# NHLBI/long_context_biomedical_imaging

Hardware: AMD Instinct MI355X
Metric: image-tokens/sec fwd+bwd, ViT patch=2 512^2 (L=65536), 1/2/4/8 MI355X (higher is better)
Workload: dtype bf16; 1 GPU; ViT-small p2 512x512 2-D seg (ViTUNETR head), full attention; global_batch=2, seq_len=65536, parallelism=ddp1, per_gpu_batch=2, optimizer=adam, loss=CrossEntropy, activation_checkpointing=none, hip_graph=False, tuned_gemms=True

## Files before the change

include/lci.h:

```cpp
#ifndef LCI_H_
#define LCI_H_

#ifdef __cplusplus
extern "C" {
#endif

#define LCI_ABI_VERSION 37
const char* lci_last_error(void);
int lci_abi_version(void);
const char* lci_build_hash(void);

int lci_attn_fwd(const void* qkv, void* out, float* lse2, float* knorm_ws, int B, int L, int H, int head_dim,
                 float scale, void* stream);
long long lci_attn_fwd_ws_bytes(int B, int L, int H);
int lci_attn_fwd_variant(int variant, const void* qkv, void* out, float* lse2, float* knorm_ws, int B, int L, int H,
                         int head_dim, float scale, void* stream);
int lci_attn_fwd_pick(int B, int L, int H, int n_cu);
int lci_attn_bwd(const void* qkv, const void* out, const void* dout, const float* lse2, void* dqkv,
                 float* delta_ws, int B, int L, int H, int head_dim, float scale, void* stream);
long long lci_attn_bwd_ws_bytes(int B, int H, int L);
int lci_attn_bwd_stage(int stage, const void* qkv, const void* out, const void* dout, const float* lse2,
                       void* dqkv, float* delta_ws, int B, int L, int H, int head_dim, float scale, void* stream);
int lci_attn_bwd_variant(int dq_variant, int stage, const void* qkv, const void* out, const void* dout,
                         const float* lse2, void* dqkv, float* delta_ws, int B, int L, int H, int head_dim,
                         float scale, void* stream);
int lci_attn_bwd_dq_pick(int B, int L, int H, int n_cu);

int lci_attn_gen_fwd(int dtype, const void* qkv, void* out, float* lse, int B, int L, int H, int head_dim,
                     float scale, void* stream);
int lci_attn_gen_bwd(int dtype, const void* qkv, const void* out, const void* dout, const float* lse, void* dqkv,
                     float* delta_ws, int B, int L, int H, int head_dim, float scale, void* stream);

long long lci_window_bias_elems(const int* geo, int has_mask);
int lci_window_bias(const float* rpb, const float* mask, void* bias, void* biasT, const int* geo, void* stream);
int lci_window_attn_fwd(const void* qkv, const float* qkv_bias, const void* biasT, int has_mask, void* out,
                        float* lse2, const int* geo, float scale, void* stream);
int lci_window_attn_bwd(const void* qkv, const float* qkv_bias, const void* bias, const void* biasT, int has_mask,
                        const void* out, const void* dout, const float* lse2, void* dqkv, float* dbias_pad,
                        float* pad_ws, void* dS, float* drpb, const int* geo, float scale, void* stream);
long long lci_window_dS_elems(const int* geo);
long long lci_window_pad_ws_elems(const int* geo);
int lci_window_bwd_needs_plain(const int* geo);
int lci_window_index_map(const int* geo, int* src_row, int* region, int* rid, int* wtype, void* stream);

int lci_window_gather(const void* src, void* dst, int elem_bytes, const int* geo, int scatter, void* stream);

int lci_conv3_fwd(const void* x, const void* w, void* y, int B, int D, int H, int W, int Cin, int Cout, int KD,
                  void* stream);
int lci_conv3_fwd_splits(long long V, int Cin, int Cout, int KD);
// ... 158 lines not shown
```

long_context_biomedical_imaging_amd/_lib.py:

```python
from __future__ import annotations

import ctypes
import os

import torch

HERE = os.path.dirname(os.path.abspath(__file__))
DEFAULT_LIB = os.path.join(HERE, "liblci.so")
LIB_PATH = os.environ.get("LCI_LIB_PATH", DEFAULT_LIB)
ABI_VERSION = 37

_P = ctypes.c_void_p
_I = ctypes.c_int
_F = ctypes.c_float
_L = ctypes.c_longlong
_D = ctypes.c_double

SIGNATURES = {
    "lci_attn_fwd": [_P, _P, _P, _P, _I, _I, _I, _I, _F, _P],
    "lci_attn_fwd_variant": [_I, _P, _P, _P, _P, _I, _I, _I, _I, _F, _P],
    "lci_attn_bwd": [_P, _P, _P, _P, _P, _P, _I, _I, _I, _I, _F, _P],
    "lci_attn_bwd_stage": [_I, _P, _P, _P, _P, _P, _P, _I, _I, _I, _I, _F, _P],
    "lci_attn_bwd_variant": [_I, _I, _P, _P, _P, _P, _P, _P, _I, _I, _I, _I, _F, _P],
    "lci_attn_gen_fwd": [_I, _P, _P, _P, _I, _I, _I, _I, _F, _P],
    "lci_attn_gen_bwd": [_I, _P, _P, _P, _P, _P, _P, _I, _I, _I, _I, _F, _P],
    "lci_patch_embed_fwd": [_P, _I, _P, _P, _P, _P, _I, _I, _I, _I, _I, _P, _P, _I, _P],
    "lci_patch_embed_bwd": [_P, _I, _P, _I, _P, _P, _P, _I, _I, _I, _I, _P, _P, _I, _P],
    "lci_selective_scan_fwd": [_I, _P, _P, _P, _P, _P, _P, _P, _P, _P, _I, _I, _I, _I, _I, _I, _P, _P, _P, _P, _P],
    "lci_selective_scan_bwd": [_I, _P, _P, _P, _P, _P, _P, _P, _P, _P, _P, _P, _P, _P, _P, _P, _I, _I, _I, _I, _I,
                               _I, _P, _P, _P, _P, _P],
    "lci_window_bias": [_P, _P, _P, _P, _P, _P],
    "lci_window_attn_fwd": [_P, _P, _P, _I, _P, _P, _P, _F, _P],
    "lci_window_attn_bwd": [_P, _P, _P, _P, _I, _P, _P, _P, _P, _P, _P, _P, _P, _P, _F, _P],
    "lci_window_index_map": [_P, _P, _P, _P, _P, _P],
    "lci_fft_twiddles": [_P, _I, _P],
    "lci_fftconv_spectrum": [_P, _P, _P, _P, _P, _I, _I, _P],
    "lci_fftconv_fwd": [_P, _P, _P, _P, _P, _P, _P, _I, _I, _I, _P],
    "lci_fftconv_bwd": [_P, _P, _P, _P, _P, _P, _P, _P, _P, _P, _P, _P, _I, _I, _I, _P],
    "lci_hyena_pre_fwd": [_I, _P, _P, _P, _P, _P, _I, _I, _I, _I, _I, _P],
    "lci_hyena_post_fwd": [_I, _P, _P, _P, _I, _I, _I, _P],
    "lci_hyena_post_bwd": [_I, _P, _P, _P, _P, _P, _I, _I, _I, _P],
    "lci_hyena_pre_bwd": [_I, _P, _P, _P, _P, _P, _P, _P, _P, _I, _I, _I, _I, _I, _P],
    "lci_dwconv_silu_fwd": [_I, _P, _P, _P, _P, _P, _P, _P, _I, _I, _I, _I, _I, _I, _I, _I, _P],
    "lci_conv3_fwd": [_P, _P, _P, _I, _I, _I, _I, _I, _I, _I, _P],
    "lci_conv3_fwd_split": [_P, _P, _P, _P, _I, _I, _I, _I, _I, _I, _I, _I, _P],
    "lci_conv3_pack_weight": [_P, _P, _I, _I, _I, _I, _I, _P],
# ... 61 lines not shown
    lib.lci_abi_version.restype = ctypes.c_int
    lib.lci_build_hash.restype = ctypes.c_char_p
    if lib.lci_abi_version() != ABI_VERSION:
        raise LciError(f"{path}: ABI version {lib.lci_abi_version()} != {ABI_VERSION} expected by this binding; "
                       "rebuild with `python -m long_context_biomedical_imaging_amd.build_lib`")
    if path == DEFAULT_LIB and os.path.isdir(os.path.join(HERE, "csrc")):
        from . import build_lib
        want, got = build_lib.source_hash(), lib.lci_build_hash().decode()
        if want != got:
            raise LciError(f"{path} is stale: built from sources {got}, the sources beside it hash to {want}; "
                           "rebuild with `python -m long_context_biomedical_imaging_amd.build_lib`")
    lib.lci_window_dS_elems.restype = ctypes.c_longlong
    lib.lci_window_dS_elems.argtypes = [_P]
    lib.lci_window_pad_ws_elems.restype = ctypes.c_longlong
    lib.lci_window_pad_ws_elems.argtypes = [_P]
    lib.lci_window_bwd_needs_plain.restype = ctypes.c_int
    lib.lci_window_bwd_needs_plain.argtypes = [_P]
    lib.lci_selective_scan_bwd_plain_dbc.restype = ctypes.c_int
    lib.lci_selective_scan_bwd_plain_dbc.argtypes = [_I, _I, _I]
    lib.lci_window_bias_elems.restype = ctypes.c_longlong
    lib.lci_window_bias_elems.argtypes = [_P, _I]
    lib.lci_attn_bwd_ws_bytes.restype = ctypes.c_longlong
    lib.lci_attn_bwd_ws_bytes.argtypes = [_I, _I, _I]
    lib.lci_attn_fwd_ws_bytes.restype = ctypes.c_longlong
    lib.lci_attn_fwd_ws_bytes.argtypes = [_I, _I, _I]
    lib.lci_attn_fwd_pick.restype = ctypes.c_int
    lib.lci_attn_fwd_pick.argtypes = [_I, _I, _I, _I]
    lib.lci_attn_bwd_dq_pick.restype = ctypes.c_int
    lib.lci_attn_bwd_dq_pick.argtypes = [_I, _I, _I, _I]
    lib.lci_conv3_fwd_splits.restype = ctypes.c_int
    lib.lci_conv3_fwd_splits.argtypes = [ctypes.c_longlong, _I, _I, _I]
    lib.lci_conv3_wgrad_splits.restype = ctypes.c_longlong
    lib.lci_conv3_wgrad_splits.argtypes = [ctypes.c_longlong, _I, _I, _I]
    lib.lci_linear_wgrad_splits.restype = ctypes.c_longlong
    lib.lci_linear_wgrad_splits.argtypes = [ctypes.c_longlong, _I, _I]
    lib.lci_gemm_bt_supported.restype = ctypes.c_int
    lib.lci_gemm_bt_supported.argtypes = [_I, _I]
    lib.lci_gemm_bt_small_supported.restype = ctypes.c_int
    lib.lci_gemm_bt_small_supported.argtypes = [_I, _I]
    lib.lci_linear_small_threads.restype = ctypes.c_int
    lib.lci_linear_small_threads.argtypes = []
    lib.lci_inorm_chunks.restype = ctypes.c_int
    lib.lci_inorm_chunks.argtypes = [ctypes.c_longlong, _I]
    lib.lci_layernorm_bwd_blocks.restype = ctypes.c_int
    lib.lci_layernorm_bwd_blocks.argtypes = [ctypes.c_longlong]
    lib.lci_hyena_filter_img_elems.restype = ctypes.c_longlong
    lib.lci_hyena_filter_img_elems.argtypes = []
    lib.lci_hyena_filter_partials.restype = ctypes.c_longlong
    lib.lci_hyena_filter_partials.argtypes = [_I, _I]
    lib.lci_fft_size.restype = ctypes.c_longlong
    lib.lci_fft_size.argtypes = [_I]
    lib.lci_dwconv_silu_bwd_part_rows.restype = ctypes.c_longlong
# ... 52 lines not shown
```

long_context_biomedical_imaging_amd/csrc/attention.hip:

```cpp
#include "common.hpp"

#include <type_traits>
#include <utility>

namespace lci {

constexpr int DH = 64;
constexpr int KT = 64;
constexpr float NEG_BIG = -1.0e30f;

struct AttnArgs {
  const bf16* q; const bf16* k; const bf16* v;
  const bf16* o; const bf16* dout;
  bf16* out;
  bf16* dk; bf16* dv;
  float* lse2;
  float* delta;
  long long bs_q, bs_k, bs_v, bs_o, bs_do, bs_out, bs_dk, bs_dv;
  int rs_q, rs_k, rs_v, rs_o, rs_do, rs_out, rs_dk, rs_dv;
  int hs;
  int H, L;
  float c;
  float scale;
};

__global__ __launch_bounds__(256) void attn_key_norm_kernel(AttnArgs a, float* knorm, int nkt) {
  const int lane = threadIdx.x & 63, t = blockIdx.x * 4 + (threadIdx.x >> 6);
  const int hh = blockIdx.y, b = blockIdx.z;
  if (t >= nkt) return;
  const int key = t * KT + lane;
  float ss = 0.f;
  if (key < a.L) {
    const bf16* kp = a.k + b * a.bs_k + (long long)key * a.rs_k + hh * a.hs;
#pragma unroll
    for (int c = 0; c < DH / 8; ++c) {
      const bf16x8 v = *(const bf16x8*)(kp + 8 * c);
#pragma unroll
      for (int j = 0; j < 8; ++j) ss += to_f32(v[j]) * to_f32(v[j]);
    }
  }
#pragma unroll
  for (int off = 32; off >= 1; off >>= 1) ss = fmaxf(ss, __shfl_xor(ss, off));
  if (lane == 0) knorm[((long long)b * a.H + hh) * nkt + t] = sqrtf(ss);
}

constexpr float SAFE_EXP2 = 64.f;
__global__ __launch_bounds__(256) void attn_bwd_delta_kernel(AttnArgs a) {
  const int tid = threadIdx.x;
  const int row = blockIdx.x * 32 + (tid >> 3), ch = tid & 7;
  const int hh = blockIdx.y, b = blockIdx.z;
  float acc = 0.f;
  if (row < a.L) {
    const bf16x8 o = *(const bf16x8*)(a.o + b * a.bs_o + (long long)row * a.rs_o + hh * a.hs + ch * 8);
    const bf16x8 d = *(const bf16x8*)(a.dout + b * a.bs_do + (long long)row * a.rs_do + hh * a.hs + ch * 8);
#pragma unroll
    for (int j = 0; j < 8; ++j) acc += to_f32(o[j]) * to_f32(d[j]);
  }
  acc += __shfl_xor(acc, 1);
  acc += __shfl_xor(acc, 2);
  acc += __shfl_xor(acc, 4);
  if (ch == 0 && row < a.L) {
    float* ws = a.delta + ((long long)b * a.H + hh) * 2 * a.L;
    ws[row] = -a.lse2[((long long)b * a.H + hh) * a.L + row];
    ws[a.L + row] = -acc;
  }
}

constexpr int HS_NW = 4;
__device__ __forceinline__ int sw128(int row, int col) {
  const int g = ((row >> 2) & 3) | (((row >> 1) & 1) << 2);
  return row * DH + ((((col >> 3) ^ g) << 3) | (col & 7));
}
__device__ __forceinline__ void hs_dma16(rsrc_t r, int voff, int soff, unsigned lds) {
  unsigned keep;
  asm volatile("s_mov_b32 %0, m0\n\ts_mov_b32 m0, %3\n\ts_nop 0\n\tbuffer_load_dwordx4 %1, %2, %4 offen lds\n\ts_mov_b32 m0, %0"
               : "=&s"(keep) : "v"(voff), "s"(r), "s"(lds), "s"(soff) : "memory");
}
__device__ __forceinline__ void hs_dma4(rsrc_t r, int voff, int soff, unsigned lds) {
  unsigned keep;
  asm volatile("s_mov_b32 %0, m0\n\ts_mov_b32 m0, %3\n\ts_nop 0\n\tbuffer_load_dword %1, %2, %4 offen lds\n\ts_mov_b32 m0, %0"
               : "=&s"(keep) : "v"(voff), "s"(r), "s"(lds), "s"(soff) : "memory");
}
__device__ __forceinline__ u32x4 hs_ld16(rsrc_t r, int voff, int soff) {
  u32x4 v;
  asm volatile("buffer_load_dwordx4 %0, %1, %2, %3 offen" : "=a"(v) : "v"(voff), "s"(r), "s"(soff) : "memory");
  return v;
}
__device__ __forceinline__ uint32_t hs_ld4(rsrc_t r, int voff, int soff) {
// ... 26 lines not shown
template <int OFF>
__device__ __forceinline__ void hs_st4(unsigned addr, uint32_t v) {
  asm volatile("ds_write_b32 %0, %1 offset:%2" ::"v"(addr), "a"(v), "i"(OFF) : "memory");
}
__device__ __forceinline__ u32x4 hs_ld16v(rsrc_t r, int voff, int soff) {
  u32x4 v;
  asm volatile("buffer_load_dwordx4 %0, %1, %2, %3 offen" : "=v"(v) : "v"(voff), "s"(r), "s"(soff) : "memory");
  return v;
}
template <int OFF>
__device__ __forceinline__ void hs_st16v(unsigned addr, const u32x4& v) {
  asm volatile("ds_write_b128 %0, %1 offset:%2" ::"v"(addr), "v"(v), "i"(OFF) : "memory");
}
template <class F, int... G>
__device__ __forceinline__ void hs_for_gaps(F&& f, std::integer_sequence<int, G...>) {
  (f(std::integral_constant<int, G>{}), ...);
}
#ifndef LCI_DKDV_PROBE
#define LCI_DKDV_PROBE 0
#endif
#ifndef LCI_DKDV_DPPRC
#define LCI_DKDV_DPPRC 0
#endif
template <int I>
__device__ __forceinline__ float hs_bcast(float x) {
  float d;
  asm volatile("v_mov_b32_dpp %0, %1 row_newbcast:%2 row_mask:0xf bank_mask:0xf" : "=v"(d) : "v"(x), "i"(I));
  return d;
}
__device__ __forceinline__ float hs_bcast_i(float x, int i) {
  switch (i & 15) {
    case 0: return hs_bcast<0>(x); case 1: return hs_bcast<1>(x); case 2: return hs_bcast<2>(x);
    case 3: return hs_bcast<3>(x); case 4: return hs_bcast<4>(x); case 5: return hs_bcast<5>(x);
    case 6: return hs_bcast<6>(x); case 7: return hs_bcast<7>(x); case 8: return hs_bcast<8>(x);
    case 9: return hs_bcast<9>(x); case 10: return hs_bcast<10>(x); case 11: return hs_bcast<11>(x);
    case 12: return hs_bcast<12>(x); case 13: return hs_bcast<13>(x); case 14: return hs_bcast<14>(x);
    default: return hs_bcast<15>(x);
  }
}
__global__ __launch_bounds__(HS_NW * 64, 1) void attn_bwd_dkdv_hs_kernel(AttnArgs a) {
  constexpr bool DPPRC = LCI_DKDV_DPPRC != 0;
  constexpr int TILE_B = KT * DH * 2;
  constexpr int SLOT_B = 2 * TILE_B;
  constexpr int RC_B = 2 * KT * 4;
  constexpr int NSLOT = 4;
  constexpr int NOPS = 5;
  static_assert((NSLOT & (NSLOT - 1)) == 0, "ring slot of tile t is t & (NSLOT - 1)");
  static_assert(NSLOT * SLOT_B == 65536, "Q / dO ring reachable by DS immediates");
  __shared__ __attribute__((aligned(16))) char smem[NSLOT * SLOT_B + NSLOT * RC_B];
  char* const rcs = smem + NSLOT * SLOT_B;
  const int tid = threadIdx.x, lane = tid & 63;
  const int wave = __builtin_amdgcn_readfirstlane(tid >> 6);
  const int hh = blockIdx.y, b = blockIdx.z;
  const int L = a.L;
  const int h = lane >> 5, r32 = lane & 31;
  const int kw0 = blockIdx.x * (HS_NW * 64) + wave * 64;
  const int nqt = (L + KT - 1) / KT;

  bf16x8 kf[2][4], vf[2][4];
  {
    const bf16* kp = a.k + b * a.bs_k + hh * a.hs;
    const bf16* vp = a.v + b * a.bs_v + hh * a.hs;
#pragma unroll
    for (int kb = 0; kb < 2; ++kb) {
      const int key = kw0 + 32 * kb + r32;
#pragma unroll
      for (int ks = 0; ks < 4; ++ks) {
        if (key < L) {
          kf[kb][ks] = *(const bf16x8*)(kp + (long long)key * a.rs_k + 16 * ks + 8 * h);
          vf[kb][ks] = *(const bf16x8*)(vp + (long long)key * a.rs_v + 16 * ks + 8 * h);
        } else {
          kf[kb][ks] = bf16x8{};
          vf[kb][ks] = bf16x8{};
        }
#pragma unroll
        for (int j = 0; j < 8; ++j) kf[kb][ks][j] = to_bf16(to_f32(kf[kb][ks][j]) * a.c);
      }
    }
  }
  hs_vmcnt<0>();
#pragma unroll
  for (int i = 0; i < 2; ++i)
#pragma unroll
    for (int j = 0; j < 4; ++j)
      { HS_TO_AGPR(kf[i][j]); HS_TO_AGPR(vf[i][j]); }

  const int rs2q = a.rs_q * 2, rs2d = a.rs_do * 2;
  const rsrc_t rq = make_rsrc(a.q + b * a.bs_q + hh * a.hs, (uint32_t)(L - 1) * (uint32_t)rs2q + DH * 2);
  const rsrc_t rd = make_rsrc(a.dout + b * a.bs_do + hh * a.hs, (uint32_t)(L - 1) * (uint32_t)rs2d + DH * 2);
  const rsrc_t rr = make_rsrc(a.delta + ((long long)b * a.H + hh) * 2 * L + (wave & 1) * L, (uint32_t)L * 4);
  const int prow = lane >> 3;
  const int pch0 = (lane & 7) ^ ((prow >> 2) | ((prow >> 1) & 1) << 2);
  const int pch1 = (lane & 7) ^ ((2 + (prow >> 2)) | ((prow >> 1) & 1) << 2);
  const int dq0 = (16 * wave + prow) * rs2q + 16 * pch0, dq1 = (16 * wave + 8 + prow) * rs2q + 16 * pch1;
  const int dd0 = (16 * wave + prow) * rs2d + 16 * pch0, dd1 = (16 * wave + 8 + prow) * rs2d + 16 * pch1;
  const unsigned lds0 = (unsigned)(uintptr_t)(LCI_LDS char*)smem;
  auto dma_op = [&](int t, int i) __attribute__((always_inline)) {
    const unsigned sb = lds0 + (unsigned)((t & (NSLOT - 1)) * SLOT_B);
    if (i == 0) hs_dma16(rq, dq0, t * KT * rs2q, sb + 2048 * wave);
    if (i == 1) hs_dma16(rq, dq1, t * KT * rs2q, sb + 2048 * wave + 1024);
    if (i == 2) hs_dma16(rd, dd0, t * KT * rs2d, sb + TILE_B + 2048 * wave);
    if (i == 3) hs_dma16(rd, dd1, t * KT * rs2d, sb + TILE_B + 2048 * wave + 1024);
    if (i == 4) hs_dma4(rr, lane * 4, t * KT * 4, lds0 + (unsigned)(NSLOT * SLOT_B + (t & (NSLOT - 1)) * RC_B +
                                                                     (wave & 1) * KT * 4));
  };
  auto dma_tile = [&](int t) __attribute__((always_inline)) {
#pragma unroll
    for (int i = 0; i < NOPS; ++i) dma_op(t, i);
  };
  unsigned q_off[4], t_off[2][2], rc_off;
#pragma unroll
  for (int ks = 0; ks < 4; ++ks) {
    q_off[ks] = 2 * sw128(r32, 16 * ks + 8 * h);
// ... 117 lines not shown
    for (int g = 0; g < 8; ++g) {
      chain_gap(g, 0, ST);
      valu_gap(g, 1, 1, 1, 0);
      if (!(g & 1)) tr_load(g >> 1, C, slot, r0);
      sgap(0, g);
    }
    mid();
#pragma unroll
    for (int g = 0; g < 8; ++g) {
      grad_gap(g, 1, C ^ 1);
      valu_gap(g, 0, 0, 1, 1);
      if (!(g & 1)) tr_load(4 + (g >> 1), C, slot, r0);
      if (DPPRC) {
        if (g == 1) xNL = rcx_load(nrc, 0, nr0);
        if (g == 3) xND = rcx_load(nrc, 1, nr0);
        if (g >= 5) bc_gap(g - 5, NST);
      }
      sgap(1, g);
    }
#pragma unroll
    for (int g = 0; g < 8; ++g) {
      chain_gap(g, 1, ST);
      valu_gap(g, 0, 1, 0, 0);
      if (g == 2) HS_KEEP(NLs[ST]);
      if (g == 6) HS_KEEP(NDs[ST]);
      if (DPPRC) bc_gap(3 + g, NST);
      if (g >= 2 && g < 6) qa[g - 2] = qrow(nslot, nr0, g - 2);
      if (g >= 6) {
        if (!DPPRC) rc_load(NLs[0], nrc, 0, nr0, g - 6);
        da[g - 6] = qrow(nslot + TILE_B, nr0, g - 6);
      }
      sgap(2, g);
    }
#pragma unroll
    for (int g = 0; g < 8; ++g) {
      grad_gap(g, 0, C);
      valu_gap(g, 1, 0, 0, 1);
      if (DPPRC) bc_gap(11 + g, NST);
      if (g < 2) { if (!DPPRC) rc_load(NLs[0], nrc, 0, nr0, g + 2); }
      else if (g < 6) { if (!DPPRC) rc_load(NDs[0], nrc, 1, nr0, g - 2); }
      else da[g - 4] = qrow(nslot + TILE_B, nr0, g - 4);
      sgap(3, g);
    }
  };

  u32x4 rsq[4];
  uint32_t rsr = 0;
  const unsigned wst = lds0 + 2048 * wave + 16 * lane;
  const unsigned wrc = lds0 + NSLOT * SLOT_B + (wave & 1) * KT * 4 + 4 * lane;
  auto ld_piece = [&](int t, int i) __attribute__((always_inline)) {
    if (i == 0) rsq[0] = hs_ld16(rq, dq0, t * KT * rs2q);
    if (i == 1) rsq[1] = hs_ld16(rq, dq1, t * KT * rs2q);
    if (i == 2) rsq[2] = hs_ld16(rd, dd0, t * KT * rs2d);
    if (i == 3) rsq[3] = hs_ld16(rd, dd1, t * KT * rs2d);
    if (i == 4) rsr = hs_ld4(rr, lane * 4, t * KT * 4);
  };
  dma_tile(0);
  ld_piece(1, 0); ld_piece(1, 1); ld_piece(1, 2); ld_piece(1, 3); ld_piece(1, 4);
  hs_vmcnt<0>();
  __syncthreads();
  NLs[0] = rcblk(rcs, 0, 0);
  NDs[0] = rcblk(rcs, 1, 0);
#pragma unroll
  for (int ks = 0; ks < 4; ++ks) {
    qa[ks] = qrow(0, 0, ks);
    da[ks] = qrow(TILE_B, 0, ks);
  }
  __builtin_amdgcn_s_waitcnt(LGKM0_WAIT);
  auto tile = [&](auto SL, int t) __attribute__((always_inline)) {
    constexpr int SLC = decltype(SL)::value;
    const int sl = SLC >= 0 ? SLC : t & (NSLOT - 1), nsl = SLC >= 0 ? (SLC + 1) & (NSLOT - 1) : (t + 1) & (NSLOT - 1);
    const int slot = sl * SLOT_B, nslot = nsl * SLOT_B, rc = sl * RC_B, nrc = nsl * RC_B;
    auto stage = [&]() __attribute__((always_inline)) {
      if (!(LCI_DKDV_PROBE & 1) && t + 1 < nqt) __builtin_amdgcn_s_barrier();
    };
    auto rstg0 = [&](int seg, int g) __attribute__((always_inline)) {
      if (!(g & 1)) return;
      constexpr int SS = 0, LS = 2;
      if (!(LCI_DKDV_PROBE & 2) && seg == SS && g == 1) hs_vmcnt<0>();
      constexpr int S1 = SLC >= 0 ? ((SLC + 1) & (NSLOT - 1)) * SLOT_B : 0;
      constexpr int R1 = SLC >= 0 ? ((SLC + 1) & (NSLOT - 1)) * RC_B : 0;
      const unsigned base = SLC >= 0 ? wst : wst + (unsigned)nslot;
      const unsigned rbase = SLC >= 0 ? wrc : wrc + (unsigned)nrc;
      if (seg == SS) {
// ... 38 lines not shown

  const float sc = a.scale;
#pragma unroll
  for (int kb = 0; kb < 2; ++kb) {
    const int key = kw0 + 32 * kb + r32;
    if (key < L) {
      bf16* dkp = a.dk + b * a.bs_dk + (long long)key * a.rs_dk + hh * a.hs;
      bf16* dvp = a.dv + b * a.bs_dv + (long long)key * a.rs_dv + hh * a.hs;
#pragma unroll
      for (int db = 0; db < 2; ++db)
#pragma unroll
        for (int g = 0; g < 4; ++g) {
          bf16x4 k4, v4;
#pragma unroll
          for (int j = 0; j < 4; ++j) {
            k4[j] = to_bf16(dk[db][kb][4 * g + j] * sc);
            v4[j] = to_bf16(dv[db][kb][4 * g + j]);
          }
          *(bf16x4*)(dkp + 32 * db + 8 * g + 4 * h) = k4;
          *(bf16x4*)(dvp + 32 * db + 8 * g + 4 * h) = v4;
        }
    }
  }
}

constexpr unsigned char DQ_SCHED[24][4] = {
    {0x28, 0x29, 0xff, 0xff},
    {0x68, 0x69, 0x2a, 0xa4},
    {0x6a, 0x2b, 0x2c, 0xff},
    {0x6b, 0x6c, 0xa5, 0x2d},
    {0x2e, 0x6d, 0x2f, 0xa6},
    {0x6e, 0x6f, 0x00, 0xa7},
    {0x01, 0x02, 0xff, 0xff},
    {0x03, 0x04, 0xff, 0xff},
    {0x05, 0x06, 0xff, 0xff},
    {0x40, 0x41, 0x42, 0x43},
    {0x80, 0x81, 0x44, 0x45},
    {0x46, 0x82, 0x07, 0x08},
    {0x47, 0x48, 0x83, 0x09},
    {0x0a, 0x49, 0x0b, 0x84},
    {0x4a, 0x4b, 0x0c, 0x85},
    {0x4c, 0x0d, 0x0e, 0xff},
    {0x4d, 0x4e, 0x86, 0x0f},
    {0x20, 0x4f, 0x21, 0x87},
    {0x22, 0x23, 0xff, 0xff},
    {0x24, 0x25, 0xff, 0xff},
// ... 1590 lines not shown
  hipLaunchKernelGGL(attn_key_norm_kernel, dim3((nkt + 3) / 4, H, B), dim3(256), 0, s, a, knorm_ws, nkt);
  LCI_LAUNCH_CHECK();
  if (variant < 0) variant = lci_attn_fwd_pick(B, L, H, attn_n_cu());
  if (variant == 1)
    hipLaunchKernelGGL(attn_fwd_hs4_kernel, dim3((L + FW4_QWG - 1) / FW4_QWG, H, B), dim3(HS_NW * 64), 0, s, a,
                       (const float*)knorm_ws);
  else
    hipLaunchKernelGGL(attn_fwd_hs_kernel, dim3((L + HS_NW * 64 - 1) / (HS_NW * 64), H, B), dim3(HS_NW * 64), 0, s, a,
                       (const float*)knorm_ws);
  LCI_LAUNCH_CHECK();
  return 0;
}

extern "C" int lci_attn_fwd(const void* qkv, void* out, float* lse2, float* knorm_ws, int B, int L, int H,
                            int head_dim, float scale, void* stream) {
  return lci_attn_fwd_variant(-1, qkv, out, lse2, knorm_ws, B, L, H, head_dim, scale, stream);
}

extern "C" long long lci_attn_bwd_ws_bytes(int B, int H, int L) {
  const long long flags = (long long)B * H * ((L + DQ4_QWG - 1) / DQ4_QWG);
  return ((dq4_flag_offset(B, H, L) + flags) * 4 + 255) / 256 * 256;
}

extern "C" int lci_attn_bwd_variant(int dq_variant, int stage, const void* qkv, const void* out, const void* dout,
                                    const float* lse2, void* dqkv, float* delta_ws, int B, int L, int H, int head_dim,
                                    float scale, void* stream) {
  LCI_CHECK(dq_variant >= -1 && dq_variant <= 1, "lci_attn_bwd_variant: dq_variant %d (want -1, 0 or 1)", dq_variant);
  LCI_CHECK(head_dim == DH, "lci_attn_bwd: head_dim %d unsupported (only 64)", head_dim);
  LCI_CHECK(B > 0 && L > 0 && H > 0, "lci_attn_bwd: bad shape B=%d L=%d H=%d", B, L, H);
  const int rs = 3 * H * DH;
  LCI_CHECK(check_packed(qkv, rs) && check_packed(dqkv, rs) && check_packed(out, H * DH) &&
                check_packed(dout, H * DH), "lci_attn_bwd: misaligned pointers");
  LCI_CHECK((long long)(L + 6 * KT) * rs * 2 < (1ll << 31), "lci_attn_bwd: L=%d too long for 32-bit buffer offsets", L);
  LCI_CHECK(delta_ws != nullptr, "lci_attn_bwd: delta_ws (lci_attn_bwd_ws_bytes) is required");
  AttnArgs a{};
  const bf16* base = (const bf16*)qkv;
  bf16* dbase = (bf16*)dqkv;
  a.q = base; a.k = base + H * DH; a.v = base + 2 * H * DH;
  a.o = (const bf16*)out; a.dout = (const bf16*)dout;
  a.lse2 = (float*)lse2; a.delta = delta_ws;
  a.bs_q = a.bs_k = a.bs_v = (long long)L * rs;
  a.rs_q = a.rs_k = a.rs_v = rs;
  a.bs_o = a.bs_do = (long long)L * H * DH;
  a.rs_o = a.rs_do = H * DH;
  a.out = dbase; a.dk = dbase + H * DH; a.dv = dbase + 2 * H * DH;
  a.bs_out = a.bs_dk = a.bs_dv = (long long)L * rs;
  a.rs_out = a.rs_dk = a.rs_dv = rs;
  a.hs = DH; a.H = H; a.L = L;
  a.scale = scale; a.c = scale * 1.4426950408889634f;
  hipStream_t s = (hipStream_t)stream;
  const dim3 grid((L + HS_NW * 64 - 1) / (HS_NW * 64), H, B);
  if (stage < 0 || stage == 0) {
    hipLaunchKernelGGL(attn_bwd_delta_kernel, dim3((L + 31) / 32, H, B), dim3(256), 0, s, a);
    LCI_LAUNCH_CHECK();
  }
  if (stage < 0 || stage == 1) {
    hipLaunchKernelGGL(attn_bwd_dkdv_hs_kernel, grid, dim3(HS_NW * 64), 0, s, a);
    LCI_LAUNCH_CHECK();
  }
  if (stage < 0 || stage == 2) {
    if (dq_variant < 0) dq_variant = lci_attn_bwd_dq_pick(B, L, H, attn_n_cu());
    if (dq_variant == 1) {
      hipLaunchKernelGGL(attn_bwd_dq_hs4_kernel, dim3((L + DQ4_QWG - 1) / DQ4_QWG, H, B), dim3(HS_NW * 64), 0, s, a);
      LCI_LAUNCH_CHECK();
      hipLaunchKernelGGL(attn_bwd_dq_hsfb_kernel, grid, dim3(HS_NW * 64), 0, s, a);
    } else {
      hipLaunchKernelGGL(attn_bwd_dq_hs_kernel, grid, dim3(HS_NW * 64), 0, s, a);
    }
    LCI_LAUNCH_CHECK();
  }
  return 0;
}

extern "C" int lci_attn_bwd_stage(int stage, const void* qkv, const void* out, const void* dout, const float* lse2,
                                  void* dqkv, float* delta_ws, int B, int L, int H, int head_dim, float scale,
                                  void* stream) {
  return lci_attn_bwd_variant(-1, stage, qkv, out, dout, lse2, dqkv, delta_ws, B, L, H, head_dim, scale, stream);
}

extern "C" int lci_attn_bwd(const void* qkv, const void* out, const void* dout, const float* lse2, void* dqkv,
                            float* delta_ws, int B, int L, int H, int head_dim, float scale, void* stream) {
  return lci_attn_bwd_stage(-1, qkv, out, dout, lse2, dqkv, delta_ws, B, L, H, head_dim, scale, stream);
}
```

long_context_biomedical_imaging_amd/kernels.py:

```python
from __future__ import annotations

import ctypes
import os

import torch

from . import _lib


class KernelTimer:
    enabled = False
    only = None
    records: list = []

    @classmethod
    def run(cls, name, work, t, fn):
        if not cls.enabled or (cls.only is not None and name not in cls.only):
            fn()
            return
        st = torch.cuda.current_stream(t.device)
        e0, e1 = torch.cuda.Event(enable_timing=True), torch.cuda.Event(enable_timing=True)
        e0.record(st)
        fn()
        e1.record(st)
# ... 35 lines not shown


def attn_fwd_variant(qkv: torch.Tensor, num_heads: int, scale: float, variant: int):
    _lib.require_gpu(qkv)
    B, L, C = qkv.shape
    dh = C // (3 * num_heads)
    if qkv.dtype != torch.bfloat16:
        raise _lib.LciError("attn_fwd_variant expects bf16 qkv")
    out = torch.empty(B, L, num_heads * dh, device=qkv.device, dtype=torch.bfloat16)
    lse2 = torch.empty(B, num_heads, L, device=qkv.device, dtype=torch.float32)
    ws = torch.empty(_lib.load().lci_attn_fwd_ws_bytes(B, L, num_heads) // 4, device=qkv.device,
                     dtype=torch.float32)
    _lib.call("lci_attn_fwd_variant", int(variant), qkv.data_ptr(), out.data_ptr(), lse2.data_ptr(), ws.data_ptr(), B,
              L, num_heads, dh, float(scale), _lib.stream_of(qkv))
    return out, lse2


def attn_bwd(qkv, out, dout, lse2, num_heads: int, scale: float):
    _lib.require_gpu(qkv, out, dout, lse2)
    B, L, C = qkv.shape
    dh = C // (3 * num_heads)
    dqkv = torch.empty_like(qkv)
    delta = torch.empty(int(_lib.load().lci_attn_bwd_ws_bytes(B, num_heads, L)), device=qkv.device, dtype=torch.uint8)
    args = (qkv.data_ptr(), out.data_ptr(), dout.data_ptr(), lse2.data_ptr(), dqkv.data_ptr(), delta.data_ptr(),
            B, L, num_heads, dh, float(scale), _lib.stream_of(qkv))
    if not KernelTimer.enabled:
        _lib.call("lci_attn_bwd", *args)
        return dqkv
    f = float(B) * num_heads * L * L * dh
    KernelTimer.run("attn_bwd_delta", 0.0, qkv, lambda: _lib.call("lci_attn_bwd_stage", 0, *args))
    KernelTimer.run("attn_bwd_dkdv", 6.0 * f, qkv, lambda: _lib.call("lci_attn_bwd_stage", 1, *args))
    KernelTimer.run("attn_bwd_dq", 2.0 * f, qkv, lambda: _lib.call("lci_attn_bwd_stage", 2, *args))
    return dqkv


def attn_bwd_variant(qkv, out, dout, lse2, num_heads: int, scale: float, dq_variant: int, stage: int = -1, ws=None,
                     dqkv=None):
    _lib.require_gpu(qkv, out, dout, lse2)
    B, L, C = qkv.shape
    dh = C // (3 * num_heads)
    if dqkv is None:
        dqkv = torch.empty_like(qkv)
    if ws is None:
        ws = torch.empty(int(_lib.load().lci_attn_bwd_ws_bytes(B, num_heads, L)) // 4, device=qkv.device,
                         dtype=torch.int32)
    _lib.call("lci_attn_bwd_variant", int(dq_variant), int(stage), qkv.data_ptr(), out.data_ptr(), dout.data_ptr(),
              lse2.data_ptr(), dqkv.data_ptr(), ws.data_ptr(), B, L, num_heads, dh, float(scale), _lib.stream_of(qkv))
    n0, nwg = B * num_heads * 2 * L, (L + 511) // 512
    return dqkv, ws[n0:n0 + B * num_heads * nwg].view(B, num_heads, nwg)


class _FlashAttention(torch.autograd.Function):
    @staticmethod
    def forward(ctx, qkv, num_heads, scale):
        out, lse2 = attn_fwd(qkv, num_heads, scale)
        ctx.save_for_backward(qkv, out, lse2)
        ctx.num_heads, ctx.scale = num_heads, scale
        return out

    @staticmethod
    def backward(ctx, dout):
        qkv, out, lse2 = ctx.saved_tensors
        dout = dout.to(torch.bfloat16).contiguous()
        return attn_bwd(qkv, out, dout, lse2, ctx.num_heads, ctx.scale), None, None


ATTN_HEAD_DIM = 64
ATTN_GEN_MAX_HEAD_DIM = 256
WIN_HEAD_DIM = 32

# ... 2036 lines not shown
```

Before: 238,500 image-tokens/s.

## Use a per-head shared softmax shift in dK/dV backward to drop per-row LSE loads

Adds a reduction kernel that computes the per-head max and min of the LSE values. When their spread fits the safe exp2 range, the delta kernel pre-scales dO and delta by exp2(c - lse) into a workspace. The dK/dV kernel then uses one constant shift in place of per-row LSE loads, which removes the rc_load traffic and broadcasts from its inner loop. The cost is an extra kernel, a second copy of dO in memory, and possible bf16 rounding and range issues when dO is rescaled.

```diff
diff --git a/include/lci.h b/include/lci.h
--- a/include/lci.h
+++ b/include/lci.h
@@ -5,7 +5,7 @@
 extern "C" {
 #endif
 
-#define LCI_ABI_VERSION 37
+#define LCI_ABI_VERSION 38
 const char* lci_last_error(void);
 int lci_abi_version(void);
 const char* lci_build_hash(void);
@@ -17,14 +17,17 @@
                          int head_dim, float scale, void* stream);
 int lci_attn_fwd_pick(int B, int L, int H, int n_cu);
 int lci_attn_bwd(const void* qkv, const void* out, const void* dout, const float* lse2, void* dqkv,
-                 float* delta_ws, int B, int L, int H, int head_dim, float scale, void* stream);
+                 float* delta_ws, void* shift_ws, int B, int L, int H, int head_dim, float scale, void* stream);
 long long lci_attn_bwd_ws_bytes(int B, int H, int L);
+long long lci_attn_bwd_shift_ws_bytes(int B, int H, int L);
 int lci_attn_bwd_stage(int stage, const void* qkv, const void* out, const void* dout, const float* lse2,
-                       void* dqkv, float* delta_ws, int B, int L, int H, int head_dim, float scale, void* stream);
-int lci_attn_bwd_variant(int dq_variant, int stage, const void* qkv, const void* out, const void* dout,
-                         const float* lse2, void* dqkv, float* delta_ws, int B, int L, int H, int head_dim,
-                         float scale, void* stream);
+                       void* dqkv, float* delta_ws, void* shift_ws, int B, int L, int H, int head_dim, float scale,
+                       void* stream);
+int lci_attn_bwd_variant(int dq_variant, int dkdv_variant, int stage, const void* qkv, const void* out,
+                         const void* dout, const float* lse2, void* dqkv, float* delta_ws, void* shift_ws, int B,
+                         int L, int H, int head_dim, float scale, void* stream);
 int lci_attn_bwd_dq_pick(int B, int L, int H, int n_cu);
+int lci_attn_bwd_dkdv_pick(int B, int L, int H);
 
 int lci_attn_gen_fwd(int dtype, const void* qkv, void* out, float* lse, int B, int L, int H, int head_dim,
                      float scale, void* stream);
diff --git a/long_context_biomedical_imaging_amd/_lib.py b/long_context_biomedical_imaging_amd/_lib.py
--- a/long_context_biomedical_imaging_amd/_lib.py
+++ b/long_context_biomedical_imaging_amd/_lib.py
@@ -8,7 +8,7 @@
 HERE = os.path.dirname(os.path.abspath(__file__))
 DEFAULT_LIB = os.path.join(HERE, "liblci.so")
 LIB_PATH = os.environ.get("LCI_LIB_PATH", DEFAULT_LIB)
-ABI_VERSION = 37
+ABI_VERSION = 38
 
 _P = ctypes.c_void_p
 _I = ctypes.c_int
@@ -19,9 +19,9 @@
 SIGNATURES = {
     "lci_attn_fwd": [_P, _P, _P, _P, _I, _I, _I, _I, _F, _P],
     "lci_attn_fwd_variant": [_I, _P, _P, _P, _P, _I, _I, _I, _I, _F, _P],
-    "lci_attn_bwd": [_P, _P, _P, _P, _P, _P, _I, _I, _I, _I, _F, _P],
-    "lci_attn_bwd_stage": [_I, _P, _P, _P, _P, _P, _P, _I, _I, _I, _I, _F, _P],
-    "lci_attn_bwd_variant": [_I, _I, _P, _P, _P, _P, _P, _P, _I, _I, _I, _I, _F, _P],
+    "lci_attn_bwd": [_P, _P, _P, _P, _P, _P, _P, _I, _I, _I, _I, _F, _P],
+    "lci_attn_bwd_stage": [_I, _P, _P, _P, _P, _P, _P, _P, _I, _I, _I, _I, _F, _P],
+    "lci_attn_bwd_variant": [_I, _I, _I, _P, _P, _P, _P, _P, _P, _P, _I, _I, _I, _I, _F, _P],
     "lci_attn_gen_fwd": [_I, _P, _P, _P, _I, _I, _I, _I, _F, _P],
     "lci_attn_gen_bwd": [_I, _P, _P, _P, _P, _P, _P, _I, _I, _I, _I, _F, _P],
     "lci_patch_embed_fwd": [_P, _I, _P, _P, _P, _P, _I, _I, _I, _I, _I, _P, _P, _I, _P],
@@ -129,12 +129,16 @@
     lib.lci_window_bias_elems.argtypes = [_P, _I]
     lib.lci_attn_bwd_ws_bytes.restype = ctypes.c_longlong
     lib.lci_attn_bwd_ws_bytes.argtypes = [_I, _I, _I]
+    lib.lci_attn_bwd_shift_ws_bytes.restype = ctypes.c_longlong
+    lib.lci_attn_bwd_shift_ws_bytes.argtypes = [_I, _I, _I]
     lib.lci_attn_fwd_ws_bytes.restype = ctypes.c_longlong
     lib.lci_attn_fwd_ws_bytes.argtypes = [_I, _I, _I]
     lib.lci_attn_fwd_pick.restype = ctypes.c_int
     lib.lci_attn_fwd_pick.argtypes = [_I, _I, _I, _I]
     lib.lci_attn_bwd_dq_pick.restype = ctypes.c_int
     lib.lci_attn_bwd_dq_pick.argtypes = [_I, _I, _I, _I]
+    lib.lci_attn_bwd_dkdv_pick.restype = ctypes.c_int
+    lib.lci_attn_bwd_dkdv_pick.argtypes = [_I, _I, _I]
     lib.lci_conv3_fwd_splits.restype = ctypes.c_int
     lib.lci_conv3_fwd_splits.argtypes = [ctypes.c_longlong, _I, _I, _I]
     lib.lci_conv3_wgrad_splits.restype = ctypes.c_longlong
diff --git a/long_context_biomedical_imaging_amd/csrc/attention.hip b/long_context_biomedical_imaging_amd/csrc/attention.hip
--- a/long_context_biomedical_imaging_amd/csrc/attention.hip
+++ b/long_context_biomedical_imaging_amd/csrc/attention.hip
@@ -16,6 +16,9 @@
   bf16* dk; bf16* dv;
   float* lse2;
   float* delta;
+  bf16* dout_s;
+  float* ndelta_s;
+  float* lmax_s; float* lmin_s;
   long long bs_q, bs_k, bs_v, bs_o, bs_do, bs_out, bs_dk, bs_dv;
   int rs_q, rs_k, rs_v, rs_o, rs_do, rs_out, rs_dk, rs_dv;
   int hs;
@@ -45,14 +48,52 @@
 }
 
 constexpr float SAFE_EXP2 = 64.f;
+constexpr int SHIFT_NP = 16;
+__global__ __launch_bounds__(256) void attn_bwd_shift_kernel(AttnArgs a) {
+  const int tid = threadIdx.x, part = blockIdx.x, hh = blockIdx.y, b = blockIdx.z;
+  const float* l2 = a.lse2 + ((long long)b * a.H + hh) * a.L;
+  const int n = (a.L + SHIFT_NP - 1) / SHIFT_NP, end = min(a.L, (part + 1) * n);
+  float mx = -3.0e38f, mn = 3.0e38f;
+  for (int i = part * n + tid; i < end; i += 256) {
+    const float v = l2[i];
+    mx = fmaxf(mx, v);
+    mn = fminf(mn, v);
+  }
+#pragma unroll
+  for (int off = 32; off >= 1; off >>= 1) {
+    mx = fmaxf(mx, __shfl_xor(mx, off));
+    mn = fminf(mn, __shfl_xor(mn, off));
+  }
+  __shared__ float wmx[4], wmn[4];
+  if ((tid & 63) == 0) { wmx[tid >> 6] = mx; wmn[tid >> 6] = mn; }
+  __syncthreads();
+  if (tid == 0) {
+    a.lmax_s[(b * a.H + hh) * SHIFT_NP + part] = fmaxf(fmaxf(wmx[0], wmx[1]), fmaxf(wmx[2], wmx[3]));
+    a.lmin_s[(b * a.H + hh) * SHIFT_NP + part] = fminf(fminf(wmn[0], wmn[1]), fminf(wmn[2], wmn[3]));
+  }
+}
+__device__ __forceinline__ float dkdv_shift_c(const AttnArgs& a, int b, int hh, bool& ok) {
+  const float* pm = a.lmax_s + (b * a.H + hh) * SHIFT_NP;
+  const float* pn = a.lmin_s + (b * a.H + hh) * SHIFT_NP;
+  float c = -3.0e38f, lo = 3.0e38f;
+#pragma unroll
+  for (int i = 0; i < SHIFT_NP; ++i) {
+    c = fmaxf(c, pm[i]);
+    lo = fminf(lo, pn[i]);
+  }
+  ok = c - lo <= SAFE_EXP2 && c >= -SAFE_EXP2 && c <= 1.0e30f;
+  return c;
+}
 __global__ __launch_bounds__(256) void attn_bwd_delta_kernel(AttnArgs a) {
   const int tid = threadIdx.x;
   const int row = blockIdx.x * 32 + (tid >> 3), ch = tid & 7;
   const int hh = blockIdx.y, b = blockIdx.z;
-  float acc = 0.f;
+  float acc = 0.f, l2 = 0.f;
+  bf16x8 d = {};
   if (row < a.L) {
     const bf16x8 o = *(const bf16x8*)(a.o + b * a.bs_o + (long long)row * a.rs_o + hh * a.hs + ch * 8);
-    const bf16x8 d = *(const bf16x8*)(a.dout + b * a.bs_do + (long long)row * a.rs_do + hh * a.hs + ch * 8);
+    d = *(const bf16x8*)(a.dout + b * a.bs_do + (long long)row * a.rs_do + hh * a.hs + ch * 8);
+    l2 = a.lse2[((long long)b * a.H + hh) * a.L + row];
 #pragma unroll
     for (int j = 0; j < 8; ++j) acc += to_f32(o[j]) * to_f32(d[j]);
   }
@@ -61,9 +102,18 @@
   acc += __shfl_xor(acc, 4);
   if (ch == 0 && row < a.L) {
     float* ws = a.delta + ((long long)b * a.H + hh) * 2 * a.L;
-    ws[row] = -a.lse2[((long long)b * a.H + hh) * a.L + row];
+    ws[row] = -l2;
     ws[a.L + row] = -acc;
   }
+  if (a.dout_s == nullptr || row >= a.L) return;
+  bool ok;
+  const float c = dkdv_shift_c(a, b, hh, ok);
+  const float f = ok ? exp2_fast(c - l2) : 1.f;
+  bf16x8 ds;
+#pragma unroll
+  for (int j = 0; j < 8; ++j) ds[j] = to_bf16(f * to_f32(d[j]));
+  *(bf16x8*)(a.dout_s + b * a.bs_do + (long long)row * a.rs_do + hh * a.hs + ch * 8) = ds;
+  if (ch == 0) a.ndelta_s[((long long)b * a.H + hh) * a.L + row] = -(f * acc);
 }
 
 constexpr int HS_NW = 4;
@@ -136,6 +186,10 @@
 #ifndef LCI_DKDV_DPPRC
 #define LCI_DKDV_DPPRC 0
 #endif
+constexpr int DKDV_TILE_B = KT * DH * 2;
+constexpr int DKDV_SLOT_B = 2 * DKDV_TILE_B;
+constexpr int DKDV_RC_B = 2 * KT * 4;
+constexpr int DKDV_NSLOT = 4;
 template <int I>
 __device__ __forceinline__ float hs_bcast(float x) {
   float d;
@@ -152,16 +206,13 @@
     default: return hs_bcast<15>(x);
   }
 }
-__global__ __launch_bounds__(HS_NW * 64, 1) void attn_bwd_dkdv_hs_kernel(AttnArgs a) {
-  constexpr bool DPPRC = LCI_DKDV_DPPRC != 0;
-  constexpr int TILE_B = KT * DH * 2;
-  constexpr int SLOT_B = 2 * TILE_B;
-  constexpr int RC_B = 2 * KT * 4;
-  constexpr int NSLOT = 4;
+template <bool SHIFT>
+__device__ __forceinline__ void attn_bwd_dkdv_hs_body(const AttnArgs& a, char* const smem) {
+  constexpr bool DPPRC = !SHIFT && LCI_DKDV_DPPRC != 0;
+  constexpr int TILE_B = DKDV_TILE_B, SLOT_B = DKDV_SLOT_B, RC_B = DKDV_RC_B, NSLOT = DKDV_NSLOT;
   constexpr int NOPS = 5;
   static_assert((NSLOT & (NSLOT - 1)) == 0, "ring slot of tile t is t & (NSLOT - 1)");
   static_assert(NSLOT * SLOT_B == 65536, "Q / dO ring reachable by DS immediates");
-  __shared__ __attribute__((aligned(16))) char smem[NSLOT * SLOT_B + NSLOT * RC_B];
   char* const rcs = smem + NSLOT * SLOT_B;
   const int tid = threadIdx.x, lane = tid & 63;
   const int wave = __builtin_amdgcn_readfirstlane(tid >> 6);
@@ -201,8 +252,10 @@
 
   const int rs2q = a.rs_q * 2, rs2d = a.rs_do * 2;
   const rsrc_t rq = make_rsrc(a.q + b * a.bs_q + hh * a.hs, (uint32_t)(L - 1) * (uint32_t)rs2q + DH * 2);
-  const rsrc_t rd = make_rsrc(a.dout + b * a.bs_do + hh * a.hs, (uint32_t)(L - 1) * (uint32_t)rs2d + DH * 2);
-  const rsrc_t rr = make_rsrc(a.delta + ((long long)b * a.H + hh) * 2 * L + (wave & 1) * L, (uint32_t)L * 4);
+  const rsrc_t rd = make_rsrc((SHIFT ? a.dout_s : a.dout) + b * a.bs_do + hh * a.hs,
+                              (uint32_t)(L - 1) * (uint32_t)rs2d + DH * 2);
+  const rsrc_t rr = SHIFT ? make_rsrc(a.ndelta_s + ((long long)b * a.H + hh) * L, (uint32_t)L * 4)
+                          : make_rsrc(a.delta + ((long long)b * a.H + hh) * 2 * L + (wave & 1) * L, (uint32_t)L * 4);
   const int prow = lane >> 3;
   const int pch0 = (lane & 7) ^ ((prow >> 2) | ((prow >> 1) & 1) << 2);
   const int pch1 = (lane & 7) ^ ((2 + (prow >> 2)) | ((prow >> 1) & 1) << 2);
@@ -366,12 +419,13 @@
     for (int g = 0; g < 8; ++g) {
       chain_gap(g, 1, ST);
       valu_gap(g, 0, 1, 0, 0);
+      if (SHIFT && g == 1) __builtin_amdgcn_s_waitcnt(LGKM0_WAIT);
       if (g == 2) HS_KEEP(NLs[ST]);
       if (g == 6) HS_KEEP(NDs[ST]);
       if (DPPRC) bc_gap(3 + g, NST);
       if (g >= 2 && g < 6) qa[g - 2] = qrow(nslot, nr0, g - 2);
       if (g >= 6) {
-        if (!DPPRC) rc_load(NLs[0], nrc, 0, nr0, g - 6);
+        if (!DPPRC && !SHIFT) rc_load(NLs[0], nrc, 0, nr0, g - 6);
         da[g - 6] = qrow(nslot + TILE_B, nr0, g - 6);
       }
       sgap(2, g);
@@ -381,9 +435,10 @@
       grad_gap(g, 0, C);
       valu_gap(g, 1, 0, 0, 1);
       if (DPPRC) bc_gap(11 + g, NST);
-      if (g < 2) { if (!DPPRC) rc_load(NLs[0], nrc, 0, nr0, g + 2); }
+      if (g < 2) { if (!DPPRC && !SHIFT) rc_load(NLs[0], nrc, 0, nr0, g + 2); }
       else if (g < 6) { if (!DPPRC) rc_load(NDs[0], nrc, 1, nr0, g - 2); }
       else da[g - 4] = qrow(nslot + TILE_B, nr0, g - 4);
+      if (SHIFT && g == 7) __builtin_amdgcn_s_waitcnt(LGKM0_WAIT | (2 << 8));
       sgap(3, g);
     }
   };
@@ -403,7 +458,15 @@
   ld_piece(1, 0); ld_piece(1, 1); ld_piece(1, 2); ld_piece(1, 3); ld_piece(1, 4);
   hs_vmcnt<0>();
   __syncthreads();
-  NLs[0] = rcblk(rcs, 0, 0);
+  if (SHIFT) {
+    bool ok;
+    const float nc = -dkdv_shift_c(a, b, hh, ok);
+#pragma unroll
+    for (int i = 0; i < 16; ++i) NLs[0][i] = nc;
+    HS_OPAQUE(NLs[0]);
+  } else {
+    NLs[0] = rcblk(rcs, 0, 0);
+  }
   NDs[0] = rcblk(rcs, 1, 0);
 #pragma unroll
   for (int ks = 0; ks < 4; ++ks) {
@@ -488,6 +551,13 @@
         }
     }
   }
+}
+__global__ __launch_bounds__(HS_NW * 64, 1) void attn_bwd_dkdv_hs_kernel(AttnArgs a) {
+  __shared__ __attribute__((aligned(16))) char smem[DKDV_NSLOT * DKDV_SLOT_B + DKDV_NSLOT * DKDV_RC_B];
+  bool shift = false;
+  if (a.dout_s != nullptr) dkdv_shift_c(a, blockIdx.z, blockIdx.y, shift);
+  if (shift) attn_bwd_dkdv_hs_body<true>(a, smem);
+  else attn_bwd_dkdv_hs_body<false>(a, smem);
 }
 
 constexpr unsigned char DQ_SCHED[24][4] = {
@@ -2124,10 +2194,19 @@
   return ((dq4_flag_offset(B, H, L) + flags) * 4 + 255) / 256 * 256;
 }
 
-extern "C" int lci_attn_bwd_variant(int dq_variant, int stage, const void* qkv, const void* out, const void* dout,
-                                    const float* lse2, void* dqkv, float* delta_ws, int B, int L, int H, int head_dim,
-                                    float scale, void* stream) {
+static long long dkdv_shift_do_bytes(int B, int H, int L) { return (long long)B * L * H * DH * 2; }
+extern "C" long long lci_attn_bwd_shift_ws_bytes(int B, int H, int L) {
+  return (dkdv_shift_do_bytes(B, H, L) + ((long long)B * H * L + 2ll * B * H * SHIFT_NP) * 4 + 255) / 256 * 256;
+}
+
+extern "C" int lci_attn_bwd_dkdv_pick(int B, int L, int H) { return B > 0 && H > 0 && L >= 32768 ? 1 : 0; }
+
+extern "C" int lci_attn_bwd_variant(int dq_variant, int dkdv_variant, int stage, const void* qkv, const void* out,
+                                    const void* dout, const float* lse2, void* dqkv, float* delta_ws, void* shift_ws,
+                                    int B, int L, int H, int head_dim, float scale, void* stream) {
   LCI_CHECK(dq_variant >= -1 && dq_variant <= 1, "lci_attn_bwd_variant: dq_variant %d (want -1, 0 or 1)", dq_variant);
+  LCI_CHECK(dkdv_variant >= -1 && dkdv_variant <= 1, "lci_attn_bwd_variant: dkdv_variant %d (want -1, 0 or 1)",
+            dkdv_variant);
   LCI_CHECK(head_dim == DH, "lci_attn_bwd: head_dim %d unsupported (only 64)", head_dim);
   LCI_CHECK(B > 0 && L > 0 && H > 0, "lci_attn_bwd: bad shape B=%d L=%d H=%d", B, L, H);
   const int rs = 3 * H * DH;
@@ -2135,6 +2214,11 @@
                 check_packed(dout, H * DH), "lci_attn_bwd: misaligned pointers");
   LCI_CHECK((long long)(L + 6 * KT) * rs * 2 < (1ll << 31), "lci_attn_bwd: L=%d too long for 32-bit buffer offsets", L);
   LCI_CHECK(delta_ws != nullptr, "lci_attn_bwd: delta_ws (lci_attn_bwd_ws_bytes) is required");
+  if (dkdv_variant < 0) dkdv_variant = lci_attn_bwd_dkdv_pick(B, L, H);
+  const bool use_shift = dkdv_variant == 1 && stage != 2;
+  LCI_CHECK(!use_shift || shift_ws != nullptr,
+            "lci_attn_bwd: shift_ws (lci_attn_bwd_shift_ws_bytes) is required by the shared-shift dK/dV stream");
+  LCI_CHECK(!use_shift || ((uintptr_t)shift_ws & 15) == 0, "lci_attn_bwd: misaligned shift_ws");
   AttnArgs a{};
   const bf16* base = (const bf16*)qkv;
   bf16* dbase = (bf16*)dqkv;
@@ -2152,12 +2236,23 @@
   a.scale = scale; a.c = scale * 1.4426950408889634f;
   hipStream_t s = (hipStream_t)stream;
   const dim3 grid((L + HS_NW * 64 - 1) / (HS_NW * 64), H, B);
+  AttnArgs as = a;
+  if (use_shift) {
+    as.dout_s = (bf16*)shift_ws;
+    as.ndelta_s = (float*)((char*)shift_ws + dkdv_shift_do_bytes(B, H, L));
+    as.lmax_s = as.ndelta_s + (long long)B * H * L;
+    as.lmin_s = as.lmax_s + (long long)B * H * SHIFT_NP;
+  }
   if (stage < 0 || stage == 0) {
-    hipLaunchKernelGGL(attn_bwd_delta_kernel, dim3((L + 31) / 32, H, B), dim3(256), 0, s, a);
+    if (use_shift) {
+      hipLaunchKernelGGL(attn_bwd_shift_kernel, dim3(SHIFT_NP, H, B), dim3(256), 0, s, as);
+      LCI_LAUNCH_CHECK();
+    }
+    hipLaunchKernelGGL(attn_bwd_delta_kernel, dim3((L + 31) / 32, H, B), dim3(256), 0, s, as);
     LCI_LAUNCH_CHECK();
   }
   if (stage < 0 || stage == 1) {
-    hipLaunchKernelGGL(attn_bwd_dkdv_hs_kernel, grid, dim3(HS_NW * 64), 0, s, a);
+    hipLaunchKernelGGL(attn_bwd_dkdv_hs_kernel, grid, dim3(HS_NW * 64), 0, s, as);
     LCI_LAUNCH_CHECK();
   }
   if (stage < 0 || stage == 2) {
@@ -2175,12 +2270,14 @@
 }
 
 extern "C" int lci_attn_bwd_stage(int stage, const void* qkv, const void* out, const void* dout, const float* lse2,
-                                  void* dqkv, float* delta_ws, int B, int L, int H, int head_dim, float scale,
-                                  void* stream) {
-  return lci_attn_bwd_variant(-1, stage, qkv, out, dout, lse2, dqkv, delta_ws, B, L, H, head_dim, scale, stream);
+                                  void* dqkv, float* delta_ws, void* shift_ws, int B, int L, int H, int head_dim,
+                                  float scale, void* stream) {
+  return lci_attn_bwd_variant(-1, -1, stage, qkv, out, dout, lse2, dqkv, delta_ws, shift_ws, B, L, H, head_dim, scale,
+                              stream);
 }
 
 extern "C" int lci_attn_bwd(const void* qkv, const void* out, const void* dout, const float* lse2, void* dqkv,
-                            float* delta_ws, int B, int L, int H, int head_dim, float scale, void* stream) {
-  return lci_attn_bwd_stage(-1, qkv, out, dout, lse2, dqkv, delta_ws, B, L, H, head_dim, scale, stream);
-}
+                            float* delta_ws, void* shift_ws, int B, int L, int H, int head_dim, float scale,
+                            void* stream) {
+  return lci_attn_bwd_stage(-1, qkv, out, dout, lse2, dqkv, delta_ws, shift_ws, B, L, H, head_dim, scale, stream);
+}
diff --git a/long_context_biomedical_imaging_amd/kernels.py b/long_context_biomedical_imaging_amd/kernels.py
--- a/long_context_biomedical_imaging_amd/kernels.py
+++ b/long_context_biomedical_imaging_amd/kernels.py
@@ -81,8 +81,10 @@
     dh = C // (3 * num_heads)
     dqkv = torch.empty_like(qkv)
     delta = torch.empty(int(_lib.load().lci_attn_bwd_ws_bytes(B, num_heads, L)), device=qkv.device, dtype=torch.uint8)
+    shift = attn_bwd_shift_ws(B, num_heads, L, qkv.device) if _lib.load().lci_attn_bwd_dkdv_pick(B, L, num_heads) \
+        else None
     args = (qkv.data_ptr(), out.data_ptr(), dout.data_ptr(), lse2.data_ptr(), dqkv.data_ptr(), delta.data_ptr(),
-            B, L, num_heads, dh, float(scale), _lib.stream_of(qkv))
+            shift.data_ptr() if shift is not None else None, B, L, num_heads, dh, float(scale), _lib.stream_of(qkv))
     if not KernelTimer.enabled:
         _lib.call("lci_attn_bwd", *args)
         return dqkv
@@ -93,8 +95,27 @@
     return dqkv
 
 
+def attn_bwd_shift_ws(B: int, num_heads: int, L: int, device):
+    return torch.empty(int(_lib.load().lci_attn_bwd_shift_ws_bytes(B, num_heads, L)), device=device, dtype=torch.uint8)
+
+
+def attn_bwd_shift_views(shift_ws, B: int, num_heads: int, L: int):
+    n_do, npart = B * L * num_heads * 64 * 2, 16
+    do_s = shift_ws[:n_do].view(torch.bfloat16).view(B, L, num_heads * 64)
+    rest = shift_ws[n_do:n_do + 4 * (B * num_heads * L + 2 * B * num_heads * npart)]
+    nd = rest[:4 * B * num_heads * L].view(torch.float32).view(B, num_heads, L)
+    ex = rest[4 * B * num_heads * L:].view(torch.float32).view(2, B, num_heads, npart)
+    return do_s, nd, ex[0], ex[1]
+
+
+def attn_bwd_shift_flags(shift_ws, B: int, num_heads: int, L: int):
+    _, _, lmax, lmin = attn_bwd_shift_views(shift_ws, B, num_heads, L)
+    c, lo = lmax.amax(-1), lmin.amin(-1)
+    return ~((c - lo <= 64.0) & (c >= -64.0) & (c <= 1.0e30))
+
+
 def attn_bwd_variant(qkv, out, dout, lse2, num_heads: int, scale: float, dq_variant: int, stage: int = -1, ws=None,
-                     dqkv=None):
+                     dqkv=None, dkdv_variant: int = -1, shift_ws=None):
     _lib.require_gpu(qkv, out, dout, lse2)
     B, L, C = qkv.shape
     dh = C // (3 * num_heads)
@@ -103,8 +124,17 @@
     if ws is None:
         ws = torch.empty(int(_lib.load().lci_attn_bwd_ws_bytes(B, num_heads, L)) // 4, device=qkv.device,
                          dtype=torch.int32)
-    _lib.call("lci_attn_bwd_variant", int(dq_variant), int(stage), qkv.data_ptr(), out.data_ptr(), dout.data_ptr(),
-              lse2.data_ptr(), dqkv.data_ptr(), ws.data_ptr(), B, L, num_heads, dh, float(scale), _lib.stream_of(qkv))
+    if dkdv_variant < 0:
+        dkdv_variant = int(_lib.load().lci_attn_bwd_dkdv_pick(B, L, num_heads))
+    if shift_ws is None and dkdv_variant == 1:
+        if stage < 0:
+            shift_ws = attn_bwd_shift_ws(B, num_heads, L, qkv.device)
+        elif stage == 0:
+            dkdv_variant = 0
+    _lib.call("lci_attn_bwd_variant", int(dq_variant), int(dkdv_variant), int(stage), qkv.data_ptr(), out.data_ptr(),
+              dout.data_ptr(), lse2.data_ptr(), dqkv.data_ptr(), ws.data_ptr(),
+              shift_ws.data_ptr() if shift_ws is not None else None, B, L, num_heads, dh, float(scale),
+              _lib.stream_of(qkv))
     n0, nwg = B * num_heads * 2 * L, (L + 511) // 512
     return dqkv, ws[n0:n0 + B * num_heads * nwg].view(B, num_heads, nwg)
 
```

Result: no change. 240,700 image-tokens/s (median of 6 runs) (+0.9%).
